# dalab/matrix-manifolds

Hardware: AMD Instinct MI355X
Metric: pairwise manifold-dist/sec (fwd+bwd), SPD(3) 5k-node (higher is better)
Workload: dtype f32; 1 GPU; grqc-class graph, n=5000 nodes -> SPD(3) affine-invariant, all 12497500 pairs, squared distance + backward, reference init (||log X||=0.1); parallelism=pair-rows sharded x1, 1 all-reduce, launch=hipGraph replay (kernels)

## Files before the change

matrix-manifolds_amd/csrc/spd_pair.hpp:

```cpp
#pragma once
#include <hip/hip_runtime.h>

#include "../../include/mm_manifolds.h"
#include "prof.hpp"
#include <algorithm>
#include <climits>
#include <cstdint>
#include <cstdlib>
#include <type_traits>

#include "smallmat.hpp"
#include "loss.hpp"
#include "adam.hpp"
#include "spd_rules.hpp"

#include "spd_ws.hpp"
#include "spd_step.hpp"
#include "stamp.hpp"

namespace mm {

template <typename T, int D>
__device__ __forceinline__ void node_tables(const T (&xs)[Packed<D>::NP], int i, T* __restrict__ nodeL, T* __restrict__ nodeX,
                                            T* __restrict__ nodeC, int* __restrict__ bad, T* __restrict__ nodeLd,
// ... 200 lines not shown
      return logsq_series3<float>(a, &e2);
    }
    if (!__any(centred_far3<float>(a))) return logsq_series3_centred<float>(a);
    eig3_trig(a, w);
    const bool wide = !(w[0] * 32.f > w[2]);
    if (__any(wide)) {
      if constexpr (CHOL) {
        float lw[3];
        return pair_core<float, 3, false, true>(li, xj, wmin, wmax, w, lw, v);
      } else {
        jacobi_eig<float, 3, false, true>(a, v, Num<float>::eps());
        w[0] = a[pidx(0, 0)]; w[1] = a[pidx(1, 1)]; w[2] = a[pidx(2, 2)];
      }
    }
    float s = 0.f;
#pragma unroll
    for (int k = 0; k < 3; ++k) {
      const float l = Num<float>::log(fminf(fmaxf(w[k], wmin), wmax));
      s = fmaf(l, l, s);
    }
    return s;
  } else if constexpr (D == 3 || D == 4) {
    constexpr int NP = Packed<D>::NP;
    T a[NP], m0[NP];
    pair_a<T, D, CHOL>(li, xj, a);
    if constexpr (D == 3) {
      if (__builtin_expect(!__any(!(close_dev3<T>(a) <= T(kCloseGate))), 1)) {
        T e2;
        return logsq_series3<T>(a, &e2);
      }
      if constexpr (HAS_LD && fwd_uses_logdet<T, D>()) {
        T gate;
        const T sc = logsq_cayley3<T>(a, logdet_a, &gate);
        if (__builtin_expect(!__any(!(gate <= T(kCayleyGate))), 1)) return sc;
        T w[D], lw[D], v[D][D];
        return pair_core<T, D, false, CHOL>(li, xj, wmin, wmax, w, lw, v);
      }
    } else {
      if (__builtin_expect(!__any(!(close_gate<T, D>(a) <= T(kCloseGate))), 1)) return logsq_series4<T>(a);
      if constexpr (std::is_same<T, float>::value) {
        if (!__any(centred_far4<T>(a))) return logsq_series4_centred<T>(a);
      }
    }
    const T gate = log_cayley<T, D>(a, m0);
    if (__builtin_expect(!__any(!(gate <= T(kCayleyGate))), 1)) return frob2<T, D>(m0);
    T w[D], lw[D], v[D][D];
    return pair_core<T, D, false, CHOL>(li, xj, wmin, wmax, w, lw, v);
  } else if constexpr (D == 2 && CHOL) {
    T mlog[3];
    return log_pair2_chol<T>(li, xj, wmin, wmax, mlog);
  } else if constexpr (D >= 5) {
    constexpr int NP = Packed<D>::NP;
    T a[NP], m0[NP];
    pair_a<T, D, CHOL>(li, xj, a);
    if (__builtin_expect(!__any(!(close_gate<T, D>(a) <= T(kCloseGate))), 1)) {
      log_close_mat<T, D>(a, m0);
      return frob2<T, D>(m0);
    }
    if (!__any(centred_far_mat<T, D>(a))) {
      log_centred_mat<T, D>(a, m0);
      return frob2<T, D>(m0);
    }
    T w[D], lw[D], v[D][D];
    return pair_core<T, D, false, CHOL>(li, xj, wmin, wmax, w, lw, v);
  } else {
    T w[D], lw[D], v[D][D];
    return pair_core<T, D, false, CHOL>(li, xj, wmin, wmax, w, lw, v);
  }
}

constexpr int kSpd2FwdNC = 2, kSpd2BwdNC = 2;
template <typename T, int D> constexpr int pair_cols() { return (sizeof(T) == 4 && D == 2) ? kSpd2FwdNC : (sizeof(T) == 4 && D <= 3) ? 2 : ((sizeof(T) == 4 && D == 4) ? MM_SPD4_FWD_NC : 1); }
template <typename T, int D> constexpr int pair_cols_bwd() { return (sizeof(T) == 4 && D == 3) ? MM_SPD3_BWD_NC : (sizeof(T) == 4 && D == 2) ? kSpd2BwdNC : ((sizeof(T) == 4 && D == 4) ? MM_SPD4_BWD_NC : 1); }

template <typename T, int D, int TI, bool SQ>
__global__ __launch_bounds__(kBlock) void spd_pdist_fwd_kernel(const T* __restrict__ nodeL,
                                                               const T* __restrict__ nodeY ,
                                                               const T* __restrict__ nodeLd , int n, int row_begin,
                                                               int row_end, T wmin, T wmax, T* __restrict__ out) {
  constexpr int NP = Packed<D>::NP;
  constexpr int NC = pair_cols<T, D>();
  constexpr bool kLd = fwd_uses_logdet<T, D>();
  static_assert(TI % 2 == 0, "the row loop is unrolled twice");
  const TileId tile = fold_tile<TI, kBlock * NC>(n, row_begin, row_end);
  if (!tile.ok) return;
  const int i0 = tile.i0, i1 = min(i0 + TI, row_end);
  const int lane = threadIdx.x & 63;
  const int wave = __builtin_amdgcn_readfirstlane(threadIdx.x >> 6);
  const int wave_j0 = tile.jbase + wave * (64 * NC);
  if (wave_j0 + 64 * NC - 1 <= i0) return;
  int jv[NC];
  unsigned joff[NC];
  T xj[NC][NP], ldj[NC];
  static_for<NC>([&](auto qc) {
    constexpr int q = decltype(qc)::value;
    const int j = wave_j0 + 64 * q + lane;
    const bool jin = j < n;
    jv[q] = jin ? j : INT32_MIN;
    asm volatile("" : "+v"(jv[q]));
    joff[q] = unsigned(j) * unsigned(sizeof(T));
#pragma unroll
    for (int k = 0; k < NP; ++k) xj[q][k] = T(0);
#pragma unroll
    for (int k = 0; k < D; ++k) xj[q][pidx(k, k)] = T(1);
    ldj[q] = T(0);
    if (jin) {
#pragma unroll
      for (int k = 0; k < NP; ++k) xj[q][k] = nodeY[size_t(j) * NP + k];
      if constexpr (kLd) ldj[q] = nodeLd[j];
    }
  });
  const int64_t base = pair_off(n, row_begin);
  char* op = reinterpret_cast<char*>(out + (pair_off(n, i0) - base - i0 - 1));
  unsigned ostep = unsigned(n - i0 - 2) * unsigned(sizeof(T));
  unsigned roff = unsigned(i0) * unsigned(NP * sizeof(T));
  T lrow[2][NP], ldrow[2] = {T(0), T(0)};
#pragma unroll
  for (int k = 0; k < NP; ++k) lrow[0][k] = nodeL[size_t(i0) * NP + k];
  if constexpr (kLd) ldrow[0] = nodeLd[i0];
  for (int ib = i0; ib < i1; ib += 2) {
#pragma unroll
    for (int u = 0; u < 2; ++u) {
      const int irow = ib + u;
      const int ieff = (u == 0 || irow < i1) ? irow : INT32_MAX;
      roff += unsigned(NP * sizeof(T));
      asm volatile("" : "+s"(roff));
      const T* rowp = reinterpret_cast<const T*>(reinterpret_cast<const char*>(nodeL) + roff);
#pragma unroll
      for (int k = 0; k < NP; ++k) lrow[u ^ 1][k] = rowp[k];
      if constexpr (kLd) ldrow[u ^ 1] = nodeLd[irow + 1];
      const T (&li)[NP] = lrow[u];
      static_for<NC>([&](auto qc) {
        constexpr int q = decltype(qc)::value;
        T s = Num<T>::max_raw_s(pair_value<T, D, true, kLd>(li, xj[q], wmin, wmax, ldj[q] - ldrow[u]), wmin);
        if constexpr (!SQ) s = Num<T>::sqrt(s);
        asm volatile("" : "+v"(joff[q]));
        if (jv[q] > ieff) *reinterpret_cast<T*>(op + joff[q]) = s;
      });
      op += ostep;
      ostep -= unsigned(sizeof(T));
    }
  }
}

template <typename T, int LOSS>
__device__ __forceinline__ T upstream_of(T loaded, T dsq, bool valid, int squared, T wmin, T sp, const LossArgs<T>& la,
                                         T& loss_acc, T& ds_acc) {
  if constexpr (LOSS == MM_LOSS_NONE) {
    if (__builtin_expect(!squared, 0)) loaded *= T(0.5) * Num<T>::rsqrt(Num<T>::max(dsq, wmin));
    return loaded;
  } else {
    T dldm;
    const T l = loss_term<T, LOSS>(sp * dsq, loaded, la, dldm);
    loss_acc += valid ? l : T(0);
    ds_acc += valid ? dldm * dsq : T(0);
    return valid ? dldm * sp : T(0);
  }
}

__device__ __forceinline__ int batch_node(const int* __restrict__ idx32, size_t k, int n_total) {
  return int(min(unsigned(idx32[2 * k]), unsigned(n_total - 1)));
}

template <typename T>
__device__ __forceinline__ T pair_row_load(const T* __restrict__ g, int n, int64_t base, int row, int j) {
  const char* grow = reinterpret_cast<const char*>(g + (pair_off(n, row) - base - row - 1));
  const unsigned off = unsigned(min(max(j, row + 1), n - 1)) * unsigned(sizeof(T));
  return *reinterpret_cast<const T*>(grow + off);
}

template <typename T, int D, int TI, int LOSS, bool SQ, int NCX = 0, bool SUB = false>
__global__ __launch_bounds__((64 * bwd_waves<T, D>()), (bwd_min_waves_nc<T, D, NCX>())) void spd_pdist_bwd_kernel(const T* __restrict__ nodeLC ,
                                                               const T* __restrict__ nodeY ,
                                                               const T* __restrict__ g, int n, int row_begin,
                                                               int row_end, T wmin, T wmax,
                                                               T* __restrict__ accM, T* __restrict__ accS,
                                                               LossArgs<T> la,
                                                               const int64_t* __restrict__ idx, int n_total,
                                                               WalkShares shares, int* __restrict__ share_tab) {
  static_assert(!SUB || LOSS != MM_LOSS_NONE, "node minibatches exist for the fused objective only");
  const int ns = SUB ? n_total : n;
  const int* idx32 = reinterpret_cast<const int*>(idx);
  constexpr int NP = Packed<D>::NP;
  constexpr int NW = bwd_waves<T, D>();
  constexpr int NC = NCX ? NCX : pair_cols_bwd<T, D>();
  constexpr int squared = SQ ? 1 : 0;
  T sp = T(1), loss_acc = T(0), ds_acc = T(0);
  loss_resolve<T, LOSS>(la);
  if constexpr (LOSS != MM_LOSS_NONE) sp = softplus_of(la.scale_raw);
  static_assert(TI % 2 == 0, "the row loop is unrolled twice");
  __shared__ T redM[NW][TI][NP];
  __shared__ T colS[NW][NC][D * D][64];
  MM_SPD_STAMP_BEGIN();
  __builtin_amdgcn_s_setprio(3);
  const ColWalk walk(n, row_begin, row_end, 64 * NC);
  int cb, r, rem;
  shares.of_cached(walk, int(blockIdx.x), share_tab, cb, r, rem);
  const int lane = threadIdx.x & 63;
  const int wave = __builtin_amdgcn_readfirstlane(threadIdx.x >> 6);
  bool red_writer;
  const int red_slot = reduce_slot<NP>(lane, red_writer);
  const int64_t base = pair_off(n, row_begin);
  MM_SPD_STAMP_MARK(0);
  const int wave_rows = (rem + NW - 1) / NW;
  constexpr int kPrioLast = 4;
  const int prio_last = max(kPrioLast, wave_rows / 10);
  const int prio_stretch = max(wave_rows - prio_last, 3) / 3;
  int rows_left = prio_stretch;
  int phase = 0;
  __shared__ T redJunk[NW][64];
  T* red_ptr = red_writer ? &redM[wave][0][red_slot] : &redJunk[wave][lane];
  const int red_step = red_writer ? NP : 0;

  while (rem > 0) {
    const int jbase = cb * (64 * NC);
    int jv[NC];
    unsigned joff[NC];
    T xj[NC][NP], accJ[NC][D][D];
    static_for<NC>([&](auto qc) {
      constexpr int q = decltype(qc)::value;
      const int j = jbase + 64 * q + lane;
      const bool jin = j < n;
      jv[q] = jin ? j : INT32_MIN;
      asm volatile("" : "+v"(jv[q]));
      joff[q] = unsigned(min(j, n - 1)) * unsigned(sizeof(T));
      int jn = j;
      if constexpr (SUB) {
        jn = batch_node(idx32, size_t(min(j, n - 1)), n_total);
        joff[q] = unsigned(jn) * unsigned(sizeof(T));
      }
#pragma unroll
      for (int k = 0; k < NP; ++k) xj[q][k] = T(0);
#pragma unroll
      for (int k = 0; k < D; ++k) xj[q][pidx(k, k)] = T(1);
      if (jin) {
#pragma unroll
        for (int k = 0; k < NP; ++k) xj[q][k] = nodeY[size_t(jn) * NP + k];
      }
#pragma unroll
      for (int rr = 0; rr < D; ++rr)
#pragma unroll
        for (int c = 0; c < D; ++c) accJ[q][rr][c] = T(0);
    });
    const int hi = walk.hi(cb);
    const int slice_cap = max(TI, int(min(int64_t(1) << 20, (int64_t(1) << 31) / (int64_t(n) * int64_t(sizeof(T))))));
    while (rem > 0 && r < hi) {
      const int chunk = int(min(int64_t(min(hi - r, rem)), int64_t(NW) * slice_cap));
      const int tw = (chunk + NW - 1) / NW;
      const int i0 = min(r + wave * tw, r + chunk), i1 = min(i0 + tw, r + chunk);
      if (i0 < i1) {
        constexpr int kAhead = 2;
        static_assert(kAhead == 2, "the one padding row of the operand table covers one masked slot: further ahead, clamp roff");
        const int first_node = SUB ? __builtin_amdgcn_readfirstlane(batch_node(idx32, size_t(i0), n_total)) : i0;
        int next_node = SUB ? __builtin_amdgcn_readfirstlane(batch_node(idx32, size_t(min(i0 + 1, n - 1)), n_total)) : 0;
        unsigned roff = unsigned(first_node) * unsigned(2 * NP * sizeof(T));
        T lrow[kAhead][2 * NP];
#pragma unroll
        for (int k = 0; k < 2 * NP; ++k) lrow[0][k] = nodeLC[size_t(first_node) * (2 * NP) + k];
        const int glast = min(i1, walk.re) - 1;
        const int64_t gk = glast - i0;
        const unsigned gmax = unsigned((gk * (n - 2) - (int64_t(i0) * gk + gk * (gk - 1) / 2)) * int64_t(sizeof(T)));
        const char* gslice = reinterpret_cast<const char*>(g + (pair_off(n, i0) - base - i0 - 1));
        unsigned goff = 0, gstep = unsigned(n - i0 - 2) * unsigned(sizeof(T));
        unsigned jslice[NC];
        static_for<NC>([&](auto qc) {
          constexpr int q = decltype(qc)::value;
          jslice[q] = max(joff[q], unsigned(i0 + 1) * unsigned(sizeof(T)));
        });
        T gq[kAhead][NC];
        int req_row = i0, req_node = first_node;
        auto request = [&](T (&dst)[NC]) __attribute__((always_inline)) {
          if constexpr (SUB) {
            const char* grow = reinterpret_cast<const char*>(g) + size_t(req_node) * size_t(n_total) * sizeof(T);
            static_for<NC>([&](auto qc) {
              constexpr int q = decltype(qc)::value;
              dst[q] = *reinterpret_cast<const T*>(grow + joff[q]);
            });
            req_row = min(req_row + 1, glast);
            req_node = __builtin_amdgcn_readfirstlane(batch_node(idx32, size_t(req_row), n_total));
          } else {
            static_for<NC>([&](auto qc) {
              constexpr int q = decltype(qc)::value;
              asm volatile("" : "+v"(jslice[q]));
              dst[q] = *reinterpret_cast<const T*>(gslice + goff + jslice[q]);
            });
            goff = min(goff + gstep, gmax);
            gstep -= unsigned(sizeof(T));
          }
        };
#pragma unroll
        for (int u = 0; u < kAhead; ++u) request(gq[u]);
        MM_SPD_STAMP_MARK(1);
        for (int s0 = i0; s0 < i1; s0 += TI) {
        const int s1 = min(s0 + TI, i1);
        for (int ib = s0; ib < s1; ib += kAhead) {
#pragma unroll
         for (int u = 0; u < kAhead; ++u) {
          const int irow = ib + u;
          const int ieff = (u == 0 || irow < s1) ? irow : INT32_MAX;
          const T (&lcur)[2 * NP] = lrow[u];
          if constexpr (SUB) {
            roff = unsigned(next_node) * unsigned(2 * NP * sizeof(T));
            next_node = __builtin_amdgcn_readfirstlane(batch_node(idx32, size_t(min(irow + 2, n - 1)), n_total));
          } else {
            roff += unsigned(2 * NP * sizeof(T));
          }
          asm volatile("" : "+s"(roff));
          const T* rowp = reinterpret_cast<const T*>(reinterpret_cast<const char*>(nodeLC) + roff);
#pragma unroll
          for (int k = 0; k < 2 * NP; ++k) lrow[(u + 1) % kAhead][k] = rowp[k];
          T li[NP], lc[NP];
#pragma unroll
          for (int k = 0; k < NP; ++k) { li[k] = lcur[k]; lc[k] = lcur[NP + k]; }
          if (__builtin_expect(--rows_left == 0, 0)) {
            ++phase;
            if (phase == 1) { __builtin_amdgcn_s_setprio(2); rows_left = prio_stretch; }
            else if (phase == 2) { __builtin_amdgcn_s_setprio(1); rows_left = max(wave_rows - prio_last - 2 * prio_stretch, 1); }
            else { __builtin_amdgcn_s_setprio(0); rows_left = INT32_MAX; }
          }
          bool valid[NC];
          T gs[NC], m[NC][NP];
          static_for<NC>([&](auto qc) {
            constexpr int q = decltype(qc)::value;
            valid[q] = jv[q] > ieff;
            gs[q] = valid[q] ? gq[u][q] : T(0);
          });
          request(gq[u]);
          constexpr bool g_first = LOSS == MM_LOSS_NONE && SQ;
          auto jacobi_path = [&](auto qc) __attribute__((always_inline)) {
            constexpr int q = decltype(qc)::value;
            T w[D], lw[D], v[D][D];
            constexpr int kSecond = (D == 4 && NC == 2) ? 2 : 1;
            const T s = pair_core<T, D, true, true, kSecond>(li, xj[q], wmin, wmax, w, lw, v);
            gs[q] = upstream_of<T, LOSS>(gs[q], s, valid[q], squared, wmin, sp, la, loss_acc, ds_acc);
            T cm[D];
#pragma unroll
            for (int k = 0; k < D; ++k) cm[k] = (gs[q] + gs[q]) * lw[k];
            vdvt<T, D>(v, cm, m[q]);
          };
          auto finish = [&](auto qc, const T (&m0)[NP], bool scaled) __attribute__((always_inline)) {
            constexpr int q = decltype(qc)::value;
            if (scaled) {
// ... 62 lines not shown
              T m0[NP];
              const T s = log_pair2_chol<T>(li, xj[q], wmin, wmax, m0);
              gs[q] = upstream_of<T, LOSS>(gs[q], s, valid[q], squared, wmin, sp, la, loss_acc, ds_acc);
              const T g2 = gs[q] + gs[q];
#pragma unroll
              for (int k = 0; k < NP; ++k) m[q][k] = g2 * m0[k];
            });
          } else if constexpr (D >= 5) {
            static_assert(NC == 1, "one column per lane for D >= 5");
            constexpr bool kWideBwd = !(std::is_same<T, double>::value && D == 8);
            T a[NP], m0[NP];
            congr_chol<T, D>(li, xj[0], a);
            bool done = false;
            if (__builtin_expect(!__any(!(close_gate<T, D>(a) <= T(kCloseGate))), 1)) {
              log_close_mat<T, D>(a, m0);
              done = true;
            } else if (kWideBwd && !__any(centred_far_mat<T, D>(a))) {
              log_centred_mat<T, D>(a, m0);
              done = true;
            }
            if (done) finish(std::integral_constant<int, 0>{}, m0, false); else jacobi_path(std::integral_constant<int, 0>{});
          } else {
            static_for<NC>([&](auto qc) { jacobi_path(qc); });
          }
          static_for<NC>([&](auto qc) {
            constexpr int q = decltype(qc)::value;
            lt_m_lt_acc<T, D>(li, lc, m[q], accJ[q]);
#pragma unroll
            for (int rr = 0; rr < D; ++rr)
#pragma unroll
              for (int c = 0; c < D; ++c) {
                asm volatile("" : "+v"(accJ[q][rr][c]));
              }
          });
          constexpr bool kFreshSums = NC >= 2 && D >= 3;
          if constexpr (kFreshSums) {
          T ms[NP];
#pragma unroll
          for (int k = 0; k < NP; ++k) {
            ms[k] = m[0][k];
            static_for<NC - 1>([&](auto qc) { ms[k] += m[decltype(qc)::value + 1][k]; });
          }
          *red_ptr = wave_reduce_transposed<NP, T>(ms, lane);
          } else {
          static_for<NC - 1>([&](auto qc) {
            constexpr int q = decltype(qc)::value + 1;
#pragma unroll
            for (int k = 0; k < NP; ++k) m[0][k] += m[q][k];
          });
          *red_ptr = wave_reduce_transposed<NP, T>(m[0], lane);
          }
          red_ptr += red_step;
         }
        }
        const int sw = s1 - s0;
        red_ptr -= red_step * ((sw + kAhead - 1) / kAhead * kAhead);
        __builtin_amdgcn_wave_barrier();
        for (int t = lane; t < sw * NP; t += 64) {
          const int k = t / sw, il = t - k * sw;
          const int node = SUB ? batch_node(idx32, size_t(s0 + il), n_total) : s0 + il;
          atomic_add(&accM[size_t(k) * ns + node], redM[wave][il][k]);
        }
        __builtin_amdgcn_wave_barrier();
        }
        MM_SPD_STAMP_MARK(2);
      }
      r += chunk;
      rem -= chunk;
    }
    static_for<NC>([&](auto qc) {
      constexpr int q = decltype(qc)::value;
#pragma unroll
      for (int rr = 0; rr < D; ++rr)
#pragma unroll
        for (int c = 0; c < D; ++c) colS[wave][q][rr * D + c][lane] = accJ[q][rr][c];
    });
    __syncthreads();
    for (int t = wave; t < NC * D * D; t += NW) {
      const int q = t / (D * D), k = t - q * (D * D);
      const int j = jbase + 64 * q + lane;
      T sum = colS[0][q][k][lane];
#pragma unroll
      for (int wv = 1; wv < NW; ++wv) sum += colS[wv][q][k][lane];
      if (j < n) {
        const int node = SUB ? batch_node(idx32, size_t(j), n_total) : j;
        atomic_add(&accS[size_t(k) * ns + node], sum);
      }
    }
    ++cb;
    r = row_begin;
    rem -= shares.cross;
    if (rem > 0) __syncthreads();
  }
  if constexpr (LOSS != MM_LOSS_NONE) {
    __shared__ T lossW[NW][2];
    const T l = wave_sum(loss_acc), d = wave_sum(ds_acc);
    if (lane == 0) { lossW[wave][0] = l; lossW[wave][1] = d; }
    __syncthreads();
    if (threadIdx.x == 0) {
      T ls = lossW[0][0], dd = lossW[0][1];
#pragma unroll
      for (int wv = 1; wv < NW; ++wv) { ls += lossW[wv][0]; dd += lossW[wv][1]; }
      const int slot = blockIdx.x & (kLossSlots - 1);
      atomic_add(&la.slots[slot], ls);
      atomic_add(&la.slots[kLossSlots + slot], dd);
    }
  }
  MM_SPD_STAMP_END();
}

template <typename T, int D>
__device__ __forceinline__ void node_gradient(const T* __restrict__ nodeL, T* __restrict__ accM, T* __restrict__ accS, int n,
                                              int i, T (&gi)[Packed<D>::NP]) {
  constexpr int NP = Packed<D>::NP;
  T li[NP], m[NP], xinv[NP], sc[D][D];
#pragma unroll
  for (int k = 0; k < NP; ++k) {
    li[k] = nodeL[size_t(i) * NP + k];
    m[k] = accM[size_t(k) * n + i];
    accM[size_t(k) * n + i] = T(0);
  }
#pragma unroll
  for (int r = 0; r < D; ++r)
#pragma unroll
    for (int c = 0; c < D; ++c) {
      sc[r][c] = accS[size_t(r * D + c) * n + i];
      accS[size_t(r * D + c) * n + i] = T(0);
    }
  congr_lower_t<T, D>(li, m, gi);
#pragma unroll
  for (int r = 0; r < D; ++r)
#pragma unroll
    for (int c = 0; c <= r; ++c) {
      T acc = T(0);
#pragma unroll
      for (int k = r; k < D; ++k) acc = Num<T>::fma(li[pidx(k, r)], li[pidx(k, c)], acc);
      xinv[pidx(r, c)] = acc;
    }
#pragma unroll
  for (int r = 0; r < D; ++r)
#pragma unroll
    for (int c = 0; c <= r; ++c) {
      T a = T(0), b = T(0);
#pragma unroll
      for (int k = 0; k < D; ++k) {
        a = Num<T>::fma(sc[r][k], xinv[pidx(k, c)], a);
        b = Num<T>::fma(sc[c][k], xinv[pidx(k, r)], b);
      }
      gi[pidx(r, c)] = T(0.5) * (a + b) - gi[pidx(r, c)];
    }
}

template <typename T, int D>
__global__ void spd_pdist_finalize_kernel(const T* __restrict__ nodeL, T* __restrict__ accM,
                                          T* __restrict__ accS, int n, T* __restrict__ grad,
                                          T* __restrict__ slots, const T* __restrict__ scale_raw,
                                          T* __restrict__ loss_out) {
  constexpr int NP = Packed<D>::NP;
  const int i = blockIdx.x * blockDim.x + threadIdx.x;
  if (slots && blockIdx.x == 0 && threadIdx.x < 64) loss_finalize<T>(slots, scale_raw, loss_out);
  if (i >= n) return;
  T gi[NP];
  node_gradient<T, D>(nodeL, accM, accS, n, i, gi);
  store_sym_full<T, D>(grad + size_t(i) * D * D, gi);
}

template <typename T, int D>
__global__ void spd_dist_fwd_kernel(const T* __restrict__ x, const T* __restrict__ y, int64_t m, int squared, T wmin,
                                    T wmax, T* __restrict__ out) {
  constexpr int NP = Packed<D>::NP;
  const int64_t k0 = int64_t(blockIdx.x) * blockDim.x + threadIdx.x;
  const bool in = k0 < m;
// ... 213 lines not shown
  T* grad;
  T* slots; const T* scale_raw; T* loss_out;
  T* scale_x; T scale_lr, scale_clip;
  T* tabL; T* tabX; T* tabC; int* bad; T* tabLd; T* tabLC;
};
template <typename T, int D, int RULE, bool FIN, bool PREP>
__global__ void spd_fused_step_kernel(T* x, int n, StepRule<T> rule, StepFuse<T> f) {
  constexpr int NP = Packed<D>::NP;
  if constexpr (FIN) {
    if (f.slots && blockIdx.x == 0 && threadIdx.x < 64) {
      loss_finalize<T>(f.slots, f.scale_raw, f.loss_out);
      if (f.scale_x && threadIdx.x == 0) {
        const T g = f.loss_out[1];
        T scale = -f.scale_lr;
        if (f.scale_clip > T(0)) scale *= Num<T>::min(f.scale_clip / Num<T>::sqrt(Num<T>::max(g * g, T(1e-8))), T(1));
        *f.scale_x = *f.scale_x + g * scale;
      }
    }
  }
  const int i0 = blockIdx.x * blockDim.x + threadIdx.x;
  const bool in = i0 < n;
  const int i = in ? i0 : 0;
  T beta2 = T(0), alpha = T(0);
  if constexpr (RULE == RULE_ADAM) adam_coeffs(rule.adam, beta2, alpha);
  T xs[NP], gs[NP], o[NP];
  load_sym_packed<T, D>(x + size_t(i) * D * D, xs);
  if constexpr (FIN) {
    if (in) {
      node_gradient<T, D>(f.nodeL, f.accM, f.accS, n, i, gs);
      store_sym_full<T, D>(f.grad + size_t(i) * D * D, gs);
    } else {
#pragma unroll
      for (int k = 0; k < NP; ++k) gs[k] = T(0);
    }
  } else {
    load_sym_packed<T, D>(f.grad + size_t(i) * D * D, gs);
  }
  if constexpr (RULE == RULE_RSGD) {
    spd_rsgd_update<T, D>(xs, gs, rule.lr, rule.max_grad_norm, rule.exact, o);
  } else if constexpr (RULE == RULE_MOMENTUM) {
    T b[NP];
    load_sym_packed<T, D>(rule.state0 + size_t(i) * D * D, b);
    spd_momentum_update<T, D>(xs, gs, b, rule.lr, rule.momentum, rule.dampening, rule.max_grad_norm, rule.exact, o);
    if (in) store_sym_full<T, D>(rule.state0 + size_t(i) * D * D, b);
  } else {
    T mo[NP];
    load_sym_packed<T, D>(rule.state0 + size_t(i) * D * D, mo);
    const T v = spd_adam_update<T, D>(xs, gs, mo, rule.state1[size_t(i) * D * D], rule.adam, beta2, alpha, o);
    if (in) {
      store_sym_full<T, D>(rule.state0 + size_t(i) * D * D, mo);
#pragma unroll
      for (int q = 0; q < D * D; ++q) rule.state1[size_t(i) * D * D + q] = v;
    }
  }
  if (in) {
    store_sym_full<T, D>(x + size_t(i) * D * D, o);
    if constexpr (PREP) node_tables<T, D>(o, i, f.tabL, f.tabX, f.tabC, f.bad, f.tabLd, f.tabLC);
  }
  if constexpr (RULE == RULE_ADAM) adam_tick(rule.adam.step, rule.adam.ticket, gridDim.x);
}

#define MM_CHECK_LAUNCH()                         \
  do {                                            \
    hipError_t e_ = hipGetLastError();            \
    if (e_ != hipSuccess) return static_cast<int>(e_); \
  } while (0)

constexpr int kNodeBlock = 128;
template <typename T, int D>
int spd_pdist_prepare(const T* x, int64_t n, Ws<T>& ws, int flags, hipStream_t st) {
  if (!(flags & MM_WS_PREPARED)) {
    spd_prep_kernel<T, D><<<dim3((n + kNodeBlock - 1) / kNodeBlock), dim3(kNodeBlock), 0, st>>>(x, int(n), ws.nodeL, ws.nodeX, ws.nodeC,
                                                                       ws.accM, ws.accS, ws.loss, ws.bad, ws.nodeLd, ws.nodeLC);
    MM_CHECK_LAUNCH();
  }
  return MM_OK;
}

constexpr int kFwdTI = 8;
template <typename T, int D, int TI>
int spd_pdist_fwd_launch(const T* nl, const T* nc, const T* nld, int64_t n, int64_t rb, int64_t re, int squared, double wmin, double wmax,
                         T* out, hipStream_t st) {
  if (!spd_clamps_supported<D, MM_LOSS_NONE>(wmin, wmax)) return MM_ERR_UNSUPPORTED;
  const dim3 grid = fold_grid<TI, kBlock * pair_cols<T, D>()>(n, rb, re);
  if (squared)
    launch_timed(PROF_SPD_FWD, spd_pdist_fwd_kernel<T, D, TI, true>, grid, dim3(kBlock), st, nl, nc, nld, int(n), int(rb), int(re),
                 T(wmin), T(wmax), out);
  else
    launch_timed(PROF_SPD_FWD, spd_pdist_fwd_kernel<T, D, TI, false>, grid, dim3(kBlock), st, nl, nc, nld, int(n), int(rb), int(re),
                 T(wmin), T(wmax), out);
  MM_CHECK_LAUNCH();
  return MM_OK;
}
template <typename T, int D>
int spd_pdist_fwd_t(const T* x, int64_t n, int64_t rb, int64_t re, int squared, double wmin, double wmax, T* out,
                    void* wsp, int flags, hipStream_t st) {
  Ws<T> ws(wsp, n, D);
  int rc = spd_pdist_prepare<T, D>(x, n, ws, flags, st);
  if (rc) return rc;
  if (re <= rb || pair_off(n, re) == pair_off(n, rb)) return MM_OK;
  const T* nl = ws.nodeL;
  const T* nc = ws.nodeC;
  if constexpr (D <= 4) {
    const dim3 g8 = fold_grid<kFwdTI, kBlock * pair_cols<T, D>()>(n, rb, re);
    if (int64_t(g8.x) * g8.y < 4 * int64_t(device_cus()))
      return spd_pdist_fwd_launch<T, D, 2>(nl, nc, ws.nodeLd, n, rb, re, squared, wmin, wmax, out, st);
  }
  return spd_pdist_fwd_launch<T, D, kFwdTI>(nl, nc, ws.nodeLd, n, rb, re, squared, wmin, wmax, out, st);
}

constexpr int kBwdTI = 16;
template <typename T> constexpr int bwd_cross_units() { return sizeof(T) == 4 ? 16 : 8; }
constexpr int64_t kSpd4TwoColPairs = 30000000;
constexpr int64_t kSpd4TwoColBandPairs = 12000000;
template <typename T, int D, int LOSS, bool SQ, int NCX = 0, bool SUB = false>
int spd_pdist_bwd_launch_sq(Ws<T>& ws, const T* g, int64_t n, int64_t rb, int64_t re, double wmin, double wmax,
                            hipStream_t st, LossArgs<T> la, const int64_t* idx = nullptr, int64_t n_total = 0) {
  if (!spd_clamps_supported<D, LOSS>(wmin, wmax)) return MM_ERR_UNSUPPORTED;
  constexpr int kThreads = 64 * bwd_waves<T, D>();
  constexpr int kCols = NCX ? NCX : pair_cols_bwd<T, D>();
  if constexpr (!SUB && NCX == 0 && sizeof(T) == 4 && D == 4 && pair_cols_bwd<T, D>() == 1) {
    static const int two = [] { const char* e = std::getenv("MM_SPD4_BWD_TWO_COLS"); return e ? (e[0] == '1' ? 1 : 0) : -1; }();
    const int64_t pairs = pair_off(n, re) - pair_off(n, rb);
    if (two == 1 || (two < 0 && (pairs >= kSpd4TwoColPairs || (pairs >= kSpd4TwoColBandPairs && re + 2048 <= n))))
      return spd_pdist_bwd_launch_sq<T, D, LOSS, SQ, 2>(ws, g, n, rb, re, wmin, wmax, st, la);
  }
  auto kernel = spd_pdist_bwd_kernel<T, D, kBwdTI, LOSS, SQ, NCX, SUB>;
  const int64_t units = ColWalk(int(n), int(rb), int(re), 64 * kCols).total();
  if (units <= 0) return MM_OK;
  int64_t grid = resident_workgroups<spd_pdist_bwd_kernel<T, D, kBwdTI, LOSS, SQ, NCX, SUB>>(kThreads);
  {
    const int64_t cus = device_cus();
    grid = std::min<int64_t>(grid, 4 * cus);
    const int64_t half = std::max<int64_t>(1, cus / 2);
    const int64_t by_rows = kCols >= 2 ? (units / 32 + half / 2) / half * half : units / 48 / cus * cus;
    if (by_rows < grid) grid = std::max<int64_t>(cus, by_rows);
  }
  static const int64_t env_grid = std::getenv("MM_SPD_BWD_GRID") ? std::atoll(std::getenv("MM_SPD_BWD_GRID")) : 0;
  if (env_grid > 0) grid = env_grid;
  grid = std::max<int64_t>(1, std::min<int64_t>(grid, (units + 7) / 8));
  dim3 g3{unsigned(grid), 1, 1};
  const T* nlc = ws.nodeLC;
  const T* nc = ws.nodeC;
  static const int env_cross = std::getenv("MM_SPD_BWD_CROSS") ? std::atoi(std::getenv("MM_SPD_BWD_CROSS")) : bwd_cross_units<T>();
  const ColWalk hw(int(n), int(rb), int(re), 64 * kCols);
  const int cross = std::min(std::max(env_cross, 0), 1024);
  const WalkShares shares(hw.total_aug(cross), grid, cross);
  launch_timed(PROF_SPD_BWD, kernel, g3, dim3(kThreads), st, nlc, nc, g, int(n), int(rb), int(re), T(wmin), T(wmax), ws.accM, ws.accS, la,
               idx, int(n_total), shares, ws.shareTab);
  MM_CHECK_LAUNCH();
  return MM_OK;
}
template <typename T, int D, int LOSS = MM_LOSS_NONE>
int spd_pdist_bwd_launch(Ws<T>& ws, const T* g, int64_t n, int64_t rb, int64_t re, int squared, double wmin, double wmax,
                         hipStream_t st, LossArgs<T> la = LossArgs<T>{nullptr, T(1), T(0), 0, nullptr}) {
  if constexpr (LOSS != MM_LOSS_NONE) return spd_pdist_bwd_launch_sq<T, D, LOSS, true>(ws, g, n, rb, re, wmin, wmax, st, la);
  else return squared ? spd_pdist_bwd_launch_sq<T, D, LOSS, true>(ws, g, n, rb, re, wmin, wmax, st, la)
                      : spd_pdist_bwd_launch_sq<T, D, LOSS, false>(ws, g, n, rb, re, wmin, wmax, st, la);
}

template <typename T, int D>
int spd_pdist_loss_t(int kind, const T* x, const T* target, const T* scale_raw, int64_t n, int64_t rb, int64_t re,
                     double alpha, double eps, int terms, const double* loss_params, double wmin, double wmax, T* loss_out, T* grad, void* wsp,
                     int flags, hipStream_t st) {
  Ws<T> ws(wsp, n, D);
  int rc = spd_pdist_prepare<T, D>(x, n, ws, flags, st);
  if (rc) return rc;
  if (re > rb && pair_off(n, re) > pair_off(n, rb)) {
    LossArgs<T> la{scale_raw, T(alpha), T(eps), terms, ws.loss, loss_params};
    if (kind == MM_LOSS_STRESS) rc = spd_pdist_bwd_launch<T, D, MM_LOSS_STRESS>(ws, target, n, rb, re, 1, wmin, wmax, st, la);
    else rc = spd_pdist_bwd_launch<T, D, MM_LOSS_QUOTIENT>(ws, target, n, rb, re, 1, wmin, wmax, st, la);
    if (rc) return rc;
  }
  spd_pdist_finalize_kernel<T, D><<<dim3((n + kNodeBlock - 1) / kNodeBlock), dim3(kNodeBlock), 0, st>>>(ws.nodeL, ws.accM, ws.accS, int(n),
                                                                               grad, ws.loss, scale_raw, loss_out);
  MM_CHECK_LAUNCH();
  return MM_OK;
}

template <typename T, int D>
int spd_pdist_loss_subset_t(int kind, const T* x, const T* dense, const T* scale_raw, int64_t n_total, const int64_t* idx, int64_t bs,
                            int64_t rb, int64_t re, double alpha, double eps, int terms, const double* loss_params, double wmin,
                            double wmax, T* loss_out, T* grad, void* wsp, int flags, hipStream_t st) {
  Ws<T> ws(wsp, n_total, D);
  int rc = spd_pdist_prepare<T, D>(x, n_total, ws, flags, st);
  if (rc) return rc;
  if (re > rb && pair_off(bs, re) > pair_off(bs, rb)) {
    LossArgs<T> la{scale_raw, T(alpha), T(eps), terms, ws.loss, loss_params};
    if (kind == MM_LOSS_STRESS)
      rc = spd_pdist_bwd_launch_sq<T, D, MM_LOSS_STRESS, true, 0, true>(ws, dense, bs, rb, re, wmin, wmax, st, la, idx, n_total);
    else
      rc = spd_pdist_bwd_launch_sq<T, D, MM_LOSS_QUOTIENT, true, 0, true>(ws, dense, bs, rb, re, wmin, wmax, st, la, idx, n_total);
    if (rc) return rc;
  }
  spd_pdist_finalize_kernel<T, D><<<dim3((n_total + kNodeBlock - 1) / kNodeBlock), dim3(kNodeBlock), 0, st>>>(ws.nodeL, ws.accM, ws.accS, int(n_total),
                                                                                     grad, ws.loss, scale_raw, loss_out);
  MM_CHECK_LAUNCH();
  return MM_OK;
}

template <typename T, int D>
int spd_pdist_bwd_t(const T* x, const T* g, int64_t n, int64_t rb, int64_t re, int squared, double wmin, double wmax,
                    T* grad, void* wsp, int flags, hipStream_t st) {
  constexpr int NP = Packed<D>::NP;
  Ws<T> ws(wsp, n, D);
  int rc = spd_pdist_prepare<T, D>(x, n, ws, flags, st);
  if (rc) return rc;
  if (re > rb && pair_off(n, re) > pair_off(n, rb)) {
    rc = spd_pdist_bwd_launch<T, D>(ws, g, n, rb, re, squared, wmin, wmax, st);
    if (rc) return rc;
  }
  spd_pdist_finalize_kernel<T, D><<<dim3((n + kNodeBlock - 1) / kNodeBlock), dim3(kNodeBlock), 0, st>>>(
      ws.nodeL, ws.accM, ws.accS, int(n), grad, static_cast<T*>(nullptr), static_cast<const T*>(nullptr),
      static_cast<T*>(nullptr));
  MM_CHECK_LAUNCH();
  return MM_OK;
}

template <typename T, int D, bool FIN>
int spd_fused_step_launch(const mm_train_step* s, Ws<T>& ws, hipStream_t st, bool fuse_scale) {
  const mm_step_param& p = s->points[0];
  const mm_step_param& q = s->scales[0];
  const int n = int(s->n);
  StepRule<T> rule{T(p.lr), T(p.momentum), T(p.dampening), T(p.max_grad_norm), p.exact, static_cast<T*>(p.state0),
                   static_cast<T*>(p.state1),
                   AdamArgs<T>{T(p.lr), T(p.beta1), T(p.beta2), T(p.adam_eps), T(p.max_grad_norm), p.nc, p.exact, p.step, p.ticket}};
  StepFuse<T> f{ws.nodeL, ws.accM, ws.accS, static_cast<T*>(p.grad),
                ws.loss, static_cast<const T*>(q.x), static_cast<T*>(s->loss_out),
// ... 72 lines not shown
```

matrix-manifolds_amd/csrc/spd_ws.hpp:

```cpp
#pragma once
#include <hip/hip_runtime.h>

#include <atomic>
#include <cstdint>

#include "../../include/mm_manifolds.h"
#include "loss.hpp"
#include "smallmat.hpp"

namespace mm {

constexpr int kBlock = 256;
constexpr int64_t kSpdMaxNodes = int64_t(1) << 22;
#ifndef MM_SPD4_BWD_WAVES
#define MM_SPD4_BWD_WAVES 4
#endif
#ifndef MM_SPD4_BWD_NC
#define MM_SPD4_BWD_NC 1
#endif
#ifndef MM_SPD4_FWD_NC
#define MM_SPD4_FWD_NC 1
#endif
#ifndef MM_SPD3_BWD_NC
#define MM_SPD3_BWD_NC 2
// ... 13 lines not shown
template <typename T, int D, int NCX> constexpr int bwd_min_waves_nc() {
  return (NCX == 2 && sizeof(T) == 4 && D == 4) ? MM_SPD4_BWD2_WAVES : bwd_min_waves<T, D>();
}
template <typename T, int D> constexpr int bwd_waves() {
  return int(sizeof(T)) * D * D * 64 * 4 <= 65536 ? 4 : (int(sizeof(T)) * D * D * 64 * 2 <= 65536 ? 2 : 1);
}
#ifndef MM_SPD_MAX_D
#define MM_SPD_MAX_D 9
#endif
constexpr int kSpdMaxD = MM_SPD_MAX_D;

__host__ __device__ inline int64_t pair_off(int64_t n, int64_t row) { return row * (2 * n - row - 1) / 2; }

constexpr int kShareTabEntries = 2048;
inline size_t vec_ws_tables_end(size_t esz, int64_t n, int mp) {
  return (esz * (size_t(n) * (mp + 1) + 2 * kLossSlots + size_t(n + 1) * mp) + 31) / 32 * 32;
}
template <typename T> struct Ws {
  int* status;
  int* bad;
  T* nodeL;
  T* nodeX;
  T* nodeC;
  T* accM;
  T* accS;
  T* loss;
  T* nodeLd;
  T* nodeLC;
  int* shareTab;
  static size_t bad_bytes(int64_t n) { return (size_t(n) * sizeof(int) + 63) / 64 * 64; }
  static size_t tables_end(int64_t n, int d) {
    const int np = d * (d + 1) / 2;
    return 64 + bad_bytes(n) + sizeof(T) * (size_t(n) * (6 * np + d * d + 1) + 2 * kLossSlots + 2 * np);
  }
  static size_t bytes(int64_t n, int d) { return (tables_end(n, d) + 31) / 32 * 32 + size_t(kShareTabEntries) * 32; }
  Ws(void* base, int64_t n, int d) {
    const int np = d * (d + 1) / 2;
    char* p = static_cast<char*>(base);
    status = reinterpret_cast<int*>(p);
    bad = reinterpret_cast<int*>(p + 64);
    nodeL = reinterpret_cast<T*>(p + 64 + bad_bytes(n));
    nodeX = nodeL + n * np;
    nodeC = nodeX + n * np;
    accM = nodeC + n * np;
    accS = accM + n * np;
    loss = accS + n * d * d;
    nodeLd = loss + 2 * kLossSlots;
    nodeLC = nodeLd + n;
    shareTab = reinterpret_cast<int*>(p + (tables_end(n, d) + 31) / 32 * 32);
  }
};

struct TileId { int i0, jbase; bool ok; };
template <int TI, int BW = kBlock> __device__ __forceinline__ TileId fold_tile(int n, int row_begin, int row_end) {
  const int gy = (row_end - row_begin + TI - 1) / TI;
  const int nJB = (n + BW - 1) / BW;
  int y = blockIdx.y, x = blockIdx.x;
  int cb0 = (row_begin + y * TI + 1) / BW;
  int cnt = nJB - cb0;
  if (x >= cnt) {
    x -= cnt;
    const int y2 = gy - 1 - y;
    if (y2 <= y) return {0, 0, false};
    y = y2;
    cb0 = (row_begin + y * TI + 1) / BW;
    cnt = nJB - cb0;
    if (x >= cnt) return {0, 0, false};
  }
  return {row_begin + y * TI, (cb0 + x) * BW, true};
}
template <int TI, int BW = kBlock> inline dim3 fold_grid(int64_t n, int64_t rb, int64_t re) {
  const int gy = int((re - rb + TI - 1) / TI);
  const int nJB = int((n + BW - 1) / BW);
  int gx = 0;
  for (int y = 0; y < (gy + 1) / 2; ++y) {
    const int y2 = gy - 1 - y;
    int c = nJB - int((rb + int64_t(y) * TI + 1) / BW);
    if (y2 > y) c += nJB - int((rb + int64_t(y2) * TI + 1) / BW);
    gx = c > gx ? c : gx;
  }
  return dim3(gx > 0 ? gx : 1, (gy + 1) / 2 > 0 ? (gy + 1) / 2 : 1);
}


struct ColWalk {
  int rb, re, ncb, c0, c1, bw;
  __host__ __device__ ColWalk(int n, int row_begin, int row_end, int block_width = 64) {
    bw = block_width;
    rb = row_begin;
    re = row_end < n - 1 ? row_end : n - 1;
    if (re < rb) re = rb;
    ncb = (n + bw - 1) / bw;
    c0 = (rb + 1) / bw;
    c1 = re / bw > c0 ? re / bw : c0;
    if (c1 > ncb) c1 = ncb;
    if (c0 > ncb) c0 = ncb;
  }
  __host__ __device__ int hi(int c) const { const int d = bw * c + bw - 1; return d < re ? d : re; }
  __host__ __device__ int64_t prefix(int c) const {
    if (c <= c0 || re == rb) return 0;
    const int64_t m = c < c1 ? c : c1;
    int64_t s = (bw / 2) * (m * (m - 1) - int64_t(c0) * (c0 - 1)) + (m - c0) * int64_t(bw - 1 - rb);
    if (c > c1) s += int64_t(c - c1) * (re - rb);
    return s;
  }
  __host__ __device__ int64_t total() const { return prefix(ncb); }
  __host__ __device__ int find(int64_t p) const {
    int lo = c0, hi_ = ncb - 1;
    while (lo < hi_) {
      const int mid = (lo + hi_ + 1) / 2;
      if (prefix(mid) <= p) lo = mid; else hi_ = mid - 1;
    }
    return lo;
  }
  static __host__ __device__ void divmod_small(int64_t total, int64_t g, int64_t& q, int64_t& r) {
    q = int64_t(double(total) / double(g));
    r = total - q * g;
    if (r < 0) { --q; r += g; } else if (r >= g) { ++q; r -= g; }
  }
  static __host__ __device__ int64_t share_begin(int64_t total, int64_t w, int64_t g) {
    int64_t q, r;
    divmod_small(total, g, q, r);
    return q * w + (w < r ? w : r);
  }
  __host__ __device__ int find_fast(int64_t p, int cross = 0) const {
    int64_t off;
    return find_fast_off(p, cross, &off);
  }
  __host__ __device__ int find_fast_off(int64_t p, int cross, int64_t* off, bool* capped = nullptr) const {
    const int last = ncb - 1;
    if (capped) *capped = false;
    if (last <= c0) { *off = p; return c0; }
    int c;
    const int64_t pc1 = aprefix(c1, cross);
    if (p >= pc1) {
      const float R = float(re - rb + cross);
      c = c1 + int(float(p - pc1) / (R > 0.f ? R : 1.f));
    } else {
      const float A = 0.5f * float(bw), Bs = A - 1.0f + float(bw * c0 - rb + cross);
      c = c0 + int((-Bs + sqrtf(Bs * Bs + 4.0f * A * float(p))) / (2.0f * A));
    }
    c = c < c0 ? c0 : (c > last ? last : c);
    int64_t P = aprefix(c, cross);
    int ku = 0, kd = 0;
    for (; ku < 4 && c < last; ++ku) {
      const int64_t L = int64_t(hi(c) - rb + cross);
      if (P + L > p) break;
      P += L;
      ++c;
    }
    for (; kd < 4 && c > c0 && P > p; ++kd) {
      --c;
      P -= int64_t(hi(c) - rb + cross);
    }
    if (__builtin_expect(ku == 4 || kd == 4, 0)) {
      if (capped) *capped = true;
      int lo = c0, hi_ = last;
#pragma nounroll
      while (lo < hi_) {
        const int mid = (lo + hi_ + 1) / 2;
        if (aprefix(mid, cross) <= p) lo = mid; else hi_ = mid - 1;
      }
      c = lo;
      P = aprefix(c, cross);
    }
    *off = p - P;
    return c;
  }
  __host__ __device__ bool find_fast_converges(int64_t p, int cross = 0) const {
    int64_t off;
    bool capped;
    find_fast_off(p, cross, &off, &capped);
    return !capped;
  }
  __host__ __device__ int64_t aprefix(int c, int cross) const { return prefix(c) + int64_t(cross) * (c > c0 ? c - c0 : 0); }
  __host__ __device__ int64_t total_aug(int cross) const { return total() + int64_t(cross) * (ncb > c0 ? ncb - c0 : 0); }
  __host__ __device__ void enter(int64_t a, int count, int cross, int* block, int* row, int* left) const {
    int64_t off;
    const int c = find_fast_off(a, cross, &off);
    *block = c;
    if (off < cross) { *row = rb; *left = count - int(cross - off); }
    else { *row = rb + int(off - cross); *left = count; }
  }
};

struct WalkShares {
  int64_t q;
  int r;
  int cross;
  WalkShares() = default;
  WalkShares(int64_t units, int64_t grid, int cross_ = 0) : q(units / grid), r(int(units % grid)), cross(cross_) {}
  __device__ __forceinline__ void of(int w, int64_t& begin, int& count) const {
    begin = q * int64_t(w) + (w < r ? w : r);
    count = int(q) + (w < r ? 1 : 0);
  }
  __device__ __forceinline__ void of(const ColWalk& walk, int w, int& block, int& row, int& left) const {
    int64_t a;
    int cnt;
    of(w, a, cnt);
    walk.enter(a, cnt, cross, &block, &row, &left);
  }
  __device__ __forceinline__ void of_cached(const ColWalk& walk, int w, int* __restrict__ tab, int& block, int& row, int& left) const {
    const bool usable = tab != nullptr && w < kShareTabEntries && r < (1 << 18) && q < (int64_t(1) << 31) && walk.ncb < (1 << 16);
    const int k4 = (r << 13) | (cross << 2) | ((walk.bw >> 6) - 1);
    const int k2 = walk.ncb | (w << 16);
    if (usable) {
      const int* e = tab + 8 * w;
      const int e0 = e[0], e1 = e[1], e2 = e[2], e3 = e[3], e4 = e[4], e5 = e[5], e6 = e[6], e7 = e[7];
      if (e0 == walk.rb && e1 == walk.re && e2 == k2 && e3 == int(q) && e4 == k4) {
        block = e5;
        row = e6;
        left = e7;
        return;
      }
    }
    of(walk, w, block, row, left);
    if (usable && threadIdx.x == 0) {
      int* e = tab + 8 * w;
      e[5] = block; e[6] = row; e[7] = left;
      e[0] = walk.rb; e[1] = walk.re; e[2] = k2; e[3] = int(q); e[4] = k4;
    }
  }
};

inline int device_cus() {
  static int cache[64] = {0};
  int dev = 0;
  if (hipGetDevice(&dev) != hipSuccess || dev < 0 || dev >= 64) dev = 0;
  if (cache[dev] == 0) {
    int cus = 0;
    if (hipDeviceGetAttribute(&cus, hipDeviceAttributeMultiprocessorCount, dev) != hipSuccess || cus < 1) cus = 256;
    cache[dev] = cus;
  }
  return cache[dev];
}

template <auto Kernel> inline int resident_workgroups(int block_threads) {
  static std::atomic<int> cache[64];
  int dev = 0;
  if (hipGetDevice(&dev) != hipSuccess || dev < 0 || dev >= 64) dev = 0;
  if (cache[dev].load(std::memory_order_relaxed) == 0) {
    int per_cu = 0, cus = 0;
    if (hipOccupancyMaxActiveBlocksPerMultiprocessor(&per_cu, Kernel, block_threads, 0) != hipSuccess || per_cu < 1) per_cu = 4;
    if (hipDeviceGetAttribute(&cus, hipDeviceAttributeMultiprocessorCount, dev) != hipSuccess || cus < 1) cus = 256;
    const int cap = (7 * 256) / block_threads > 0 ? (7 * 256) / block_threads : 1;
    if (per_cu > cap) per_cu = cap;
    cache[dev].store(per_cu * cus, std::memory_order_relaxed);
  }
  return cache[dev].load(std::memory_order_relaxed);
}

}
```

Measured before the change: 160.6 billion pairs/s.

## Right-align column blocks so the partial block falls at the diagonal

Shifts the column tiling of the SPD pairwise forward and backward kernels by the remainder of n modulo the block width. Block boundaries then align with the right edge, and the partial (masked) block sits at low column indices near the diagonal instead of at the far right of every row. The aim is fewer wasted lanes in the full column tiles that every row traverses. The cost is negative-index masking, clamped loads, and rewritten grid and walk helpers that must stay consistent with the output offset arithmetic.

New measurement: 162.3 billion pairs/s (median of 6 runs). 1.0% higher.

```diff
diff --git a/matrix-manifolds_amd/csrc/spd_pair.hpp b/matrix-manifolds_amd/csrc/spd_pair.hpp
--- a/matrix-manifolds_amd/csrc/spd_pair.hpp
+++ b/matrix-manifolds_amd/csrc/spd_pair.hpp
@@ -306,7 +306,7 @@
   constexpr int NC = pair_cols<T, D>();
   constexpr bool kLd = fwd_uses_logdet<T, D>();
   static_assert(TI % 2 == 0, "the row loop is unrolled twice");
-  const TileId tile = fold_tile<TI, kBlock * NC>(n, row_begin, row_end);
+  const TileId tile = fold_tile_right<TI, kBlock * NC>(n, row_begin, row_end);
   if (!tile.ok) return;
   const int i0 = tile.i0, i1 = min(i0 + TI, row_end);
   const int lane = threadIdx.x & 63;
@@ -319,7 +319,7 @@
   static_for<NC>([&](auto qc) {
     constexpr int q = decltype(qc)::value;
     const int j = wave_j0 + 64 * q + lane;
-    const bool jin = j < n;
+    const bool jin = right_col_in(j, n);
     jv[q] = jin ? j : INT32_MIN;
     asm volatile("" : "+v"(jv[q]));
     joff[q] = unsigned(j) * unsigned(sizeof(T));
@@ -417,9 +417,13 @@
   __shared__ T colS[NW][NC][D * D][64];
   MM_SPD_STAMP_BEGIN();
   __builtin_amdgcn_s_setprio(3);
-  const ColWalk walk(n, row_begin, row_end, 64 * NC);
+  const int vshift = right_shift(n, 64 * NC);
+  const ColWalk walk = right_walk(n, row_begin, row_end, 64 * NC);
+  const int walk_re = walk.re - vshift;
   int cb, r, rem;
   shares.of_cached(walk, int(blockIdx.x), share_tab, cb, r, rem);
+  r -= vshift;
+  int jbase = right_col0(cb, 64 * NC, vshift);
   const int lane = threadIdx.x & 63;
   const int wave = __builtin_amdgcn_readfirstlane(threadIdx.x >> 6);
   bool red_writer;
@@ -437,20 +441,19 @@
   const int red_step = red_writer ? NP : 0;
 
   while (rem > 0) {
-    const int jbase = cb * (64 * NC);
     int jv[NC];
     unsigned joff[NC];
     T xj[NC][NP], accJ[NC][D][D];
     static_for<NC>([&](auto qc) {
       constexpr int q = decltype(qc)::value;
       const int j = jbase + 64 * q + lane;
-      const bool jin = j < n;
+      const bool jin = right_col_in(j, n);
       jv[q] = jin ? j : INT32_MIN;
       asm volatile("" : "+v"(jv[q]));
-      joff[q] = unsigned(min(j, n - 1)) * unsigned(sizeof(T));
+      joff[q] = unsigned(min(max(j, 0), n - 1)) * unsigned(sizeof(T));
       int jn = j;
       if constexpr (SUB) {
-        jn = batch_node(idx32, size_t(min(j, n - 1)), n_total);
+        jn = batch_node(idx32, size_t(min(max(j, 0), n - 1)), n_total);
         joff[q] = unsigned(jn) * unsigned(sizeof(T));
       }
 #pragma unroll
@@ -466,7 +469,7 @@
 #pragma unroll
         for (int c = 0; c < D; ++c) accJ[q][rr][c] = T(0);
     });
-    const int hi = walk.hi(cb);
+    const int hi = right_hi(jbase, 64 * NC, walk_re);
     const int slice_cap = max(TI, int(min(int64_t(1) << 20, (int64_t(1) << 31) / (int64_t(n) * int64_t(sizeof(T))))));
     while (rem > 0 && r < hi) {
       const int chunk = int(min(int64_t(min(hi - r, rem)), int64_t(NW) * slice_cap));
@@ -481,7 +484,7 @@
         T lrow[kAhead][2 * NP];
 #pragma unroll
         for (int k = 0; k < 2 * NP; ++k) lrow[0][k] = nodeLC[size_t(first_node) * (2 * NP) + k];
-        const int glast = min(i1, walk.re) - 1;
+        const int glast = min(i1, walk_re) - 1;
         const int64_t gk = glast - i0;
         const unsigned gmax = unsigned((gk * (n - 2) - (int64_t(i0) * gk + gk * (gk - 1) / 2)) * int64_t(sizeof(T)));
         const char* gslice = reinterpret_cast<const char*>(g + (pair_off(n, i0) - base - i0 - 1));
@@ -710,12 +713,12 @@
       T sum = colS[0][q][k][lane];
 #pragma unroll
       for (int wv = 1; wv < NW; ++wv) sum += colS[wv][q][k][lane];
-      if (j < n) {
+      if (right_col_in(j, n)) {
         const int node = SUB ? batch_node(idx32, size_t(j), n_total) : j;
         atomic_add(&accS[size_t(k) * ns + node], sum);
       }
     }
-    ++cb;
+    jbase += 64 * NC;
     r = row_begin;
     rem -= shares.cross;
     if (rem > 0) __syncthreads();
@@ -1095,7 +1098,7 @@
 int spd_pdist_fwd_launch(const T* nl, const T* nc, const T* nld, int64_t n, int64_t rb, int64_t re, int squared, double wmin, double wmax,
                          T* out, hipStream_t st) {
   if (!spd_clamps_supported<D, MM_LOSS_NONE>(wmin, wmax)) return MM_ERR_UNSUPPORTED;
-  const dim3 grid = fold_grid<TI, kBlock * pair_cols<T, D>()>(n, rb, re);
+  const dim3 grid = fold_grid_right<TI, kBlock * pair_cols<T, D>()>(n, rb, re);
   if (squared)
     launch_timed(PROF_SPD_FWD, spd_pdist_fwd_kernel<T, D, TI, true>, grid, dim3(kBlock), st, nl, nc, nld, int(n), int(rb), int(re),
                  T(wmin), T(wmax), out);
@@ -1115,7 +1118,7 @@
   const T* nl = ws.nodeL;
   const T* nc = ws.nodeC;
   if constexpr (D <= 4) {
-    const dim3 g8 = fold_grid<kFwdTI, kBlock * pair_cols<T, D>()>(n, rb, re);
+    const dim3 g8 = fold_grid_right<kFwdTI, kBlock * pair_cols<T, D>()>(n, rb, re);
     if (int64_t(g8.x) * g8.y < 4 * int64_t(device_cus()))
       return spd_pdist_fwd_launch<T, D, 2>(nl, nc, ws.nodeLd, n, rb, re, squared, wmin, wmax, out, st);
   }
@@ -1139,7 +1142,8 @@
       return spd_pdist_bwd_launch_sq<T, D, LOSS, SQ, 2>(ws, g, n, rb, re, wmin, wmax, st, la);
   }
   auto kernel = spd_pdist_bwd_kernel<T, D, kBwdTI, LOSS, SQ, NCX, SUB>;
-  const int64_t units = ColWalk(int(n), int(rb), int(re), 64 * kCols).total();
+  const ColWalk hw = right_walk(int(n), int(rb), int(re), 64 * kCols);
+  const int64_t units = hw.total();
   if (units <= 0) return MM_OK;
   int64_t grid = resident_workgroups<spd_pdist_bwd_kernel<T, D, kBwdTI, LOSS, SQ, NCX, SUB>>(kThreads);
   {
@@ -1156,7 +1160,6 @@
   const T* nlc = ws.nodeLC;
   const T* nc = ws.nodeC;
   static const int env_cross = std::getenv("MM_SPD_BWD_CROSS") ? std::atoi(std::getenv("MM_SPD_BWD_CROSS")) : bwd_cross_units<T>();
-  const ColWalk hw(int(n), int(rb), int(re), 64 * kCols);
   const int cross = std::min(std::max(env_cross, 0), 1024);
   const WalkShares shares(hw.total_aug(cross), grid, cross);
   launch_timed(PROF_SPD_BWD, kernel, g3, dim3(kThreads), st, nlc, nc, g, int(n), int(rb), int(re), T(wmin), T(wmax), ws.accM, ws.accS, la,
diff --git a/matrix-manifolds_amd/csrc/spd_ws.hpp b/matrix-manifolds_amd/csrc/spd_ws.hpp
--- a/matrix-manifolds_amd/csrc/spd_ws.hpp
+++ b/matrix-manifolds_amd/csrc/spd_ws.hpp
@@ -119,6 +119,50 @@
   return dim3(gx > 0 ? gx : 1, (gy + 1) / 2 > 0 ? (gy + 1) / 2 : 1);
 }
 
+__host__ __device__ inline int right_shift(int n, int bw) {
+  const int m = n % bw;
+  return m ? bw - m : 0;
+}
+__host__ __device__ inline int right_col0(int cb, int bw, int s) { return cb * bw - s; }
+__host__ __device__ inline bool right_col_in(int j, int n) { return unsigned(j) < unsigned(n); }
+__host__ __device__ inline int right_hi(int j0, int bw, int re_real) {
+  const int d = j0 + bw - 1;
+  return d < re_real ? d : re_real;
+}
+template <int TI, int BW> __host__ __device__ inline TileId fold_tile_right_at(int n, int row_begin, int row_end, int x, int y) {
+  const int s = right_shift(n, BW);
+  const int gy = (row_end - row_begin + TI - 1) / TI;
+  const int nJB = (n + s) / BW;
+  int cb0 = (row_begin + y * TI + 1 + s) / BW;
+  int cnt = nJB - cb0;
+  if (x >= cnt) {
+    x -= cnt;
+    const int y2 = gy - 1 - y;
+    if (y2 <= y) return {0, 0, false};
+    y = y2;
+    cb0 = (row_begin + y * TI + 1 + s) / BW;
+    cnt = nJB - cb0;
+    if (x >= cnt) return {0, 0, false};
+  }
+  return {row_begin + y * TI, right_col0(cb0 + x, BW, s), true};
+}
+template <int TI, int BW> __device__ __forceinline__ TileId fold_tile_right(int n, int row_begin, int row_end) {
+  return fold_tile_right_at<TI, BW>(n, row_begin, row_end, int(blockIdx.x), int(blockIdx.y));
+}
+template <int TI, int BW> inline dim3 fold_grid_right(int64_t n, int64_t rb, int64_t re) {
+  const int s = right_shift(int(n), BW);
+  const int gy = int((re - rb + TI - 1) / TI);
+  const int nJB = int((n + s) / BW);
+  int gx = 0;
+  for (int y = 0; y < (gy + 1) / 2; ++y) {
+    const int y2 = gy - 1 - y;
+    int c = nJB - int((rb + int64_t(y) * TI + 1 + s) / BW);
+    if (y2 > y) c += nJB - int((rb + int64_t(y2) * TI + 1 + s) / BW);
+    gx = c > gx ? c : gx;
+  }
+  return dim3(gx > 0 ? gx : 1, (gy + 1) / 2 > 0 ? (gy + 1) / 2 : 1);
+}
+
 
 struct ColWalk {
   int rb, re, ncb, c0, c1, bw;
@@ -220,6 +264,10 @@
     else { *row = rb + int(off - cross); *left = count; }
   }
 };
+__host__ __device__ inline ColWalk right_walk(int n, int row_begin, int row_end, int bw) {
+  const int s = right_shift(n, bw);
+  return ColWalk(n + s, row_begin + s, (row_end < n ? row_end : n) + s, bw);
+}
 
 struct WalkShares {
   int64_t q;
```
